# IXarea/LittleGAN

Measured on AMD Instinct MI355X. Metric: 128x128 CelebA-shaped images/sec (G+D+Adj step), higher is better.
Workload: dtype bf16; 1 GPU; C3: 128x128x3 synthetic CelebA, batch 256/GPU, bf16 MFMA conv/transposed-conv + Adjuster branch; global_batch=256, per_gpu_batch=256, image=128, cond_dim=40, parallelism=dp1, launch=eager launches

## Files before the change

### littlegan_amd/csrc/heads.hip

```cpp
#include "lg_internal.h"

namespace {

constexpr int HC_MAX = 40;

__device__ __forceinline__ float head_w(const float* __restrict__ wpr, const float* __restrict__ wc, int k, int j, int c) {
  return j == 0 ? wpr[k] : wc[(long long)k * c + (j - 1)];
}

constexpr int FS = 16;
constexpr int FKC = 256;

__global__ __launch_bounds__(256) void heads_fwd_kernel(const float* __restrict__ x, const float* __restrict__ wpr,
                                                        const float* __restrict__ wc, float* __restrict__ part, int B,
                                                        int K, int c) {
  __shared__ __attribute__((aligned(16))) float xs[FS][FKC];
  __shared__ float sred[4][FS][64];
  const int lane = threadIdx.x & 63, wid = threadIdx.x >> 6;
  const int b0 = blockIdx.y * FS, k0 = blockIdx.x * FKC;
  const bool act = lane <= c;
#pragma unroll
  for (int i = 0; i < FS * FKC / 4 / 256; ++i) {
    const int q = threadIdx.x + 256 * i, b = q / (FKC / 4), k4 = (q % (FKC / 4)) * 4;
    f32x4 v = {0.f, 0.f, 0.f, 0.f};
    if (b0 + b < B && k0 + k4 < K) v = *reinterpret_cast<const f32x4*>(x + (long long)(b0 + b) * K + k0 + k4);
    *reinterpret_cast<f32x4*>(&xs[b][k4]) = v;
  }
  __syncthreads();
  float acc[FS];
#pragma unroll
  for (int s = 0; s < FS; ++s) acc[s] = 0.f;
  const int kw = wid * 64;
#pragma unroll 2
  for (int kk = 0; kk < 64; kk += 4) {
    float w[4];
#pragma unroll
    for (int e = 0; e < 4; ++e) {
      const int k = k0 + kw + kk + e;
      w[e] = (act && k < K) ? head_w(wpr, wc, k, lane, c) : 0.f;
    }
#pragma unroll
    for (int s = 0; s < FS; ++s) {
      const f32x4 xv = *reinterpret_cast<const f32x4*>(&xs[s][kw + kk]);
      acc[s] += (xv[0] * w[0] + xv[1] * w[1]) + (xv[2] * w[2] + xv[3] * w[3]);
    }
  }
#pragma unroll
  for (int s = 0; s < FS; ++s) sred[wid][s][lane] = acc[s];
  __syncthreads();
  for (int i = threadIdx.x; i < FS * 64; i += 256) {
    const int s = i >> 6, j = i & 63;
    if (j <= c && b0 + s < B)
      part[((long long)blockIdx.x * B + b0 + s) * (c + 1) + j] = (sred[0][s][j] + sred[1][s][j]) + (sred[2][s][j] + sred[3][s][j]);
  }
}

__global__ __launch_bounds__(256) void heads_final_kernel(const float* __restrict__ part, const float* __restrict__ bpr,
                                                          const float* __restrict__ bc, float* __restrict__ p, int B,
                                                          int c, int nkc) {
  const int i = blockIdx.x * 256 + threadIdx.x;
  const int n = B * (c + 1);
  if (i >= n) return;
  const int j = i % (c + 1);
  float z = 0.f;
  for (int q = 0; q < nkc; ++q) z += part[(long long)q * n + i];
  z += j == 0 ? bpr[0] : bc[j - 1];
  p[i] = 1.f / (1.f + expf(-z));
}

constexpr int DB = 16;
__global__ __launch_bounds__(256) void heads_dgrad_kernel(const float* __restrict__ dz, const float* __restrict__ wpr,
                                                          const float* __restrict__ wc, float* __restrict__ dx, int B,
                                                          int K, int c) {
  extern __shared__ __attribute__((aligned(16))) float dsm[];
  const int cp = c | 1;
  float* sw = dsm;
  float* sdz = dsm + ((256 * cp + 3) / 4) * 4;
  const int b0 = blockIdx.y * DB, k0 = blockIdx.x * 256;
  const int kn = min(256, K - k0);
  {
    const int dq = 256 / c, dr = 256 - dq * c;
    int row = threadIdx.x / c, col = threadIdx.x - row * c;
    for (int i = threadIdx.x; i < kn * c; i += 256) {
      sw[row * cp + col] = wc[(long long)k0 * c + i];
      row += dq; col += dr;
      if (col >= c) { col -= c; ++row; }
    }
  }
  for (int i = threadIdx.x; i < DB * (c + 1); i += 256) {
    const int b = i / (c + 1), j = i - b * (c + 1);
    sdz[j * DB + b] = (b0 + b < B) ? dz[(long long)(b0 + b) * (c + 1) + j] : 0.f;
  }
  __syncthreads();
  const int k = k0 + threadIdx.x;
  if (k >= K) return;
  float acc[DB];
  const float wp = wpr[k];
#pragma unroll
  for (int q = 0; q < DB / 4; ++q) {
    const f32x4 d = *reinterpret_cast<const f32x4*>(sdz + q * 4);
#pragma unroll
    for (int e = 0; e < 4; ++e) acc[q * 4 + e] = d[e] * wp;
  }
  const float* wr = sw + threadIdx.x * cp;
  for (int j = 0; j < c; ++j) {
    const float wv = wr[j];
#pragma unroll
    for (int q = 0; q < DB / 4; ++q) {
      const f32x4 d = *reinterpret_cast<const f32x4*>(sdz + (1 + j) * DB + q * 4);
#pragma unroll
      for (int e = 0; e < 4; ++e) acc[q * 4 + e] += d[e] * wv;
    }
  }
#pragma unroll
  for (int b = 0; b < DB; ++b)
    if (b0 + b < B) dx[(long long)(b0 + b) * K + k] = acc[b];
}

constexpr int WK = 64;

__global__ __launch_bounds__(256) void heads_wgrad_kernel(const float* __restrict__ x, const float* __restrict__ dz,
                                                          float* __restrict__ dwpr, float* __restrict__ dbpr,
                                                          float* __restrict__ dwc, float* __restrict__ dbc, int B, int K,
                                                          int c, int accumulate) {
  constexpr int J = HC_MAX + 1;
  __shared__ float red[J + 1][WK + 1];
  const int lane = threadIdx.x & 63;
  const int wid = __builtin_amdgcn_readfirstlane(threadIdx.x >> 6);
  const int k0 = blockIdx.x * WK, k = k0 + lane;
  const bool kok = k < K;
  const int bq = (B + 3) / 4, bs = wid * bq, be = min(B, bs + bq);
  const bool do_bias = blockIdx.x == 0;
  float acc[J];
#pragma unroll
  for (int j = 0; j < J; ++j) acc[j] = 0.f;
  float bsum = 0.f;
  constexpr int U = 8;
  for (int b = bs; b < be; b += U) {
    float xv[U], dv[U];
#pragma unroll
    for (int u = 0; u < U; ++u) {
      const bool ok = b + u < be;
      xv[u] = (ok && kok) ? x[(long long)(b + u) * K + k] : 0.f;
      dv[u] = (ok && lane <= c) ? dz[(long long)(b + u) * (c + 1) + lane] : 0.f;
    }
#pragma unroll
    for (int u = 0; u < U; ++u) {
      bsum += dv[u];
#pragma unroll
      for (int j = 0; j < J; ++j)
        acc[j] += xv[u] * __builtin_bit_cast(float, __builtin_amdgcn_readlane(__builtin_bit_cast(int, dv[u]), j));
    }
  }
  for (int w = 0; w < 4; ++w) {
    if (wid == w) {
#pragma unroll
      for (int j = 0; j < J; ++j) red[j][lane] = (w == 0 ? 0.f : red[j][lane]) + acc[j];
      red[J][lane] = (w == 0 ? 0.f : red[J][lane]) + bsum;
    }
    __syncthreads();
  }
  if (do_bias && threadIdx.x <= c) {
    float* o = threadIdx.x == 0 ? dbpr : dbc + (threadIdx.x - 1);
    *o = (accumulate ? *o : 0.f) + red[J][threadIdx.x];
  }
  for (int i = threadIdx.x; i < WK * (c + 1); i += 256) {
    const int kk = i / (c + 1), j = i - kk * (c + 1);
    if (k0 + kk < K) {
      float* o = j == 0 ? dwpr + (k0 + kk) : dwc + (long long)(k0 + kk) * c + (j - 1);
      *o = (accumulate ? *o : 0.f) + red[j][kk];
    }
  }
}

}

extern "C" size_t lg_heads_fwd_workspace_bytes(int B, int K, int c) {
  return (size_t)lg_cdiv(K, FKC) * (size_t)B * (size_t)(c + 1) * sizeof(float);
}

extern "C" int lg_heads_fwd_partials(const float* x, const float* wpr, const float* wc, float* part, int B, int K, int c, int* nkc_out,
                                     void* stream) {
  int nkc = lg_cdiv(K, FKC);
  const int rc = lg_heads_fwd_mfma_try(x, wpr, wc, part, B, K, c, &nkc, stream);
  if (rc != LG_OK && rc != LG_ERR_UNSUPPORTED) return rc;
  if (rc == LG_ERR_UNSUPPORTED) {
    hipLaunchKernelGGL(heads_fwd_kernel, dim3(nkc, lg_cdiv(B, FS)), dim3(256), 0, (hipStream_t)stream, x, wpr, wc, part,
                       B, K, c);
    LG_CHECK_LAUNCH("lg_heads_fwd");
    lg_note_kernel("heads_fwd_kernel");
  }
  *nkc_out = nkc;
  return LG_OK;
}

extern "C" int lg_heads_fwd(const float* x, const float* wpr, const float* bpr, const float* wc, const float* bc,
                            float* p, void* workspace, size_t ws_bytes, int B, int K, int c, void* stream) {
  LG_CHECK_ARG(x && wpr && bpr && wc && bc && p && workspace, "lg_heads_fwd: null pointer");
  LG_CHECK_ARG(B > 0 && K > 0 && K % 4 == 0 && c >= 1 && c <= HC_MAX, "lg_heads_fwd: bad shape B=%d K=%d c=%d", B, K, c);
  LG_CHECK_ARG(ws_bytes >= lg_heads_fwd_workspace_bytes(B, K, c), "lg_heads_fwd: workspace too small (%zu bytes)", ws_bytes);
  int nkc = 0;
  float* part = (float*)workspace;
  const int rc = lg_heads_fwd_partials(x, wpr, wc, part, B, K, c, &nkc, stream);
  if (rc != LG_OK) return rc;
  hipLaunchKernelGGL(heads_final_kernel, dim3(lg_cdiv(B * (c + 1), 256)), dim3(256), 0, (hipStream_t)stream, part, bpr,
                     bc, p, B, c, nkc);
  LG_CHECK_LAUNCH("lg_heads_fwd(final)");
  return LG_OK;
}

extern "C" int lg_heads_dgrad(const float* dz, const float* wpr, const float* wc, float* dx, int B, int K, int c,
                              void* stream) {
  LG_CHECK_ARG(dz && wpr && wc && dx, "lg_heads_dgrad: null pointer");
  LG_CHECK_ARG(B > 0 && K > 0 && c >= 1 && c <= HC_MAX, "lg_heads_dgrad: bad shape B=%d K=%d c=%d", B, K, c);
  {
    const int rc = lg_heads_dgrad_mfma_try(dz, wpr, wc, dx, B, K, c, stream);
    if (rc != LG_ERR_UNSUPPORTED) return rc;
  }
  dim3 grid(lg_cdiv(K, 256), lg_cdiv(B, DB));
  const size_t lds = (size_t)((256 * (c | 1) + 3) / 4 * 4 + DB * (c + 1)) * sizeof(float);
  hipLaunchKernelGGL(heads_dgrad_kernel, grid, dim3(256), lds, (hipStream_t)stream, dz, wpr, wc, dx, B, K, c);
  LG_CHECK_LAUNCH("lg_heads_dgrad");
  lg_note_kernel("heads_dgrad_kernel");
  return LG_OK;
}

extern "C" int lg_heads_wgrad(const float* x, const float* dz, float* dwpr, float* dbpr, float* dwc, float* dbc, int B,
                              int K, int c, int accumulate, void* stream) {
  LG_CHECK_ARG(x && dz && dwpr && dbpr && dwc && dbc, "lg_heads_wgrad: null pointer");
  LG_CHECK_ARG(B > 0 && K > 0 && K % 4 == 0 && c >= 1 && c <= HC_MAX, "lg_heads_wgrad: bad shape B=%d K=%d c=%d", B, K, c);
  {
    const int rc = lg_heads_wgrad_mfma_try(x, dz, dwpr, dbpr, dwc, dbc, B, K, c, accumulate, stream);
    if (rc != LG_ERR_UNSUPPORTED) return rc;
  }
  hipLaunchKernelGGL(heads_wgrad_kernel, dim3(lg_cdiv(K, WK)), dim3(256), 0, (hipStream_t)stream, x, dz, dwpr, dbpr,
                     dwc, dbc, B, K, c, accumulate);
  LG_CHECK_LAUNCH("lg_heads_wgrad");
  lg_note_kernel("heads_wgrad_kernel");
  return LG_OK;
}
```

### littlegan_amd/csrc/skinny_mfma.hip

```cpp
#include <stdlib.h>
#include "lg_internal.h"

namespace {

__device__ __forceinline__ f32x16 mfma2(float a, float b, f32x16 c) { return __builtin_amdgcn_mfma_f32_32x32x2f32(a, b, c, 0, 0, 0); }
__device__ __forceinline__ f32x16 zero16() {
  f32x16 z;
#pragma unroll
  for (int e = 0; e < 16; ++e) z[e] = 0.f;
  return z;
}
struct HeadCol { const float* ptr; int stride; bool ok; };
__device__ __forceinline__ HeadCol head_col(const float* wpr, const float* wc, int j, int c) {
  HeadCol h;
  h.ok = j <= c;
  h.ptr = j == 0 ? wpr : wc + (h.ok ? j - 1 : 0);
  h.stride = j == 0 ? 1 : c;
  return h;
}

__global__ __launch_bounds__(256) void heads_fwd_mfma_kernel(const float* __restrict__ x, const float* __restrict__ wpr,
                                                             const float* __restrict__ wc, float* __restrict__ part, int B,
                                                             int K, int c) {
  __shared__ float sred[4][2][16][64];
  const int lane = threadIdx.x & 63, wid = threadIdx.x >> 6, r = lane & 31, h = lane >> 5;
  const int b0 = blockIdx.y * 32, kw = blockIdx.x * 512 + wid * 128 + 8 * h;
  const float* xr = x + (long long)(b0 + r) * K + kw;
  const HeadCol c0 = head_col(wpr, wc, r, c), c1 = head_col(wpr, wc, 32 + r, c);
  const bool two = c >= 32;
  f32x16 acc0 = zero16(), acc1 = zero16();
  constexpr int GU = 2;
  for (int g2 = 0; g2 < 8; g2 += GU) {
    f32x4 alo[GU], ahi[GU];
    float w0[GU][8], w1[GU][8];
#pragma unroll
    for (int u = 0; u < GU; ++u) {
      const int g = g2 + u;
      alo[u] = *reinterpret_cast<const f32x4*>(xr + 16 * g); ahi[u] = *reinterpret_cast<const f32x4*>(xr + 16 * g + 4);
#pragma unroll
      for (int e = 0; e < 8; ++e) {
        const long long k = kw + 16 * g + e;
        w0[u][e] = c0.ok ? c0.ptr[k * c0.stride] : 0.f;
        w1[u][e] = (two && c1.ok) ? c1.ptr[k * c1.stride] : 0.f;
      }
    }
#pragma unroll
    for (int u = 0; u < GU; ++u)
#pragma unroll
      for (int e = 0; e < 8; ++e) {
        const float a = e < 4 ? alo[u][e & 3] : ahi[u][e & 3];
        acc0 = mfma2(a, w0[u][e], acc0);
        if (two) acc1 = mfma2(a, w1[u][e], acc1);
      }
  }
#pragma unroll
  for (int e = 0; e < 16; ++e) { sred[wid][0][e][lane] = acc0[e]; sred[wid][1][e][lane] = acc1[e]; }
  __syncthreads();
  for (int i = threadIdx.x; i < 32 * 64; i += 256) {
    const int row = i >> 6, j = i & 63;
    if (j <= c) {
      const int nt = j >> 5, rr = j & 31, hh = (row >> 2) & 1, e = (row & 3) + 4 * (row >> 3), l = hh * 32 + rr;
      part[((long long)blockIdx.x * B + b0 + row) * (c + 1) + j] =
          (sred[0][nt][e][l] + sred[1][nt][e][l]) + (sred[2][nt][e][l] + sred[3][nt][e][l]);
    }
  }
}

__global__ __launch_bounds__(256) void heads_wgrad_mfma_kernel(const float* __restrict__ x, const float* __restrict__ dz,
                                                              float* __restrict__ dwpr, float* __restrict__ dbpr,
                                                              float* __restrict__ dwc, float* __restrict__ dbc, int B, int K,
                                                              int c, int accumulate) {
  __shared__ float red[2][16][64];
  __shared__ float rbias[2][64];
  const int lane = threadIdx.x & 63, wid = threadIdx.x >> 6, r = lane & 31, h = lane >> 5;
  const int k0 = blockIdx.x * 32;
  const bool ok0 = r <= c, ok1 = 32 + r <= c, two = c >= 32;
  float bs0 = 0.f, bs1 = 0.f;
  const int bq = B / 4, bs = wid * bq;
  const float* xp = x + (long long)(bs + h) * K + k0 + r;
  const float* d0 = dz + (long long)(bs + h) * (c + 1) + r;
  const float* d1 = d0 + 32;
  f32x16 acc0 = zero16(), acc1 = zero16();
  constexpr int SU = 16;
  for (int b = 0; b < bq; b += 2 * SU) {
    float a[SU], v0[SU], v1[SU];
#pragma unroll
    for (int s = 0; s < SU; ++s) {
      const bool ok = b + 2 * s < bq;
      a[s] = ok ? xp[(long long)(b + 2 * s) * K] : 0.f;
      v0[s] = (ok && ok0) ? d0[(long long)(b + 2 * s) * (c + 1)] : 0.f;
      v1[s] = (ok && two && ok1) ? d1[(long long)(b + 2 * s) * (c + 1)] : 0.f;
    }
#pragma unroll
    for (int s = 0; s < SU; ++s) {
      acc0 = mfma2(a[s], v0[s], acc0);
      if (two) acc1 = mfma2(a[s], v1[s], acc1);
      bs0 += v0[s]; bs1 += v1[s];
    }
  }
  for (int w = 0; w < 4; ++w) {
    if (wid == w) {
#pragma unroll
      for (int e = 0; e < 16; ++e) {
        red[0][e][lane] = (w == 0 ? 0.f : red[0][e][lane]) + acc0[e];
        red[1][e][lane] = (w == 0 ? 0.f : red[1][e][lane]) + acc1[e];
      }
      rbias[0][lane] = (w == 0 ? 0.f : rbias[0][lane]) + bs0;
      rbias[1][lane] = (w == 0 ? 0.f : rbias[1][lane]) + bs1;
    }
    __syncthreads();
  }
  for (int i = threadIdx.x; i < 32 * 64; i += 256) {
    const int row = i >> 6, j = i & 63;
    if (j <= c) {
      const int nt = j >> 5, rr = j & 31, hh = (row >> 2) & 1, e = (row & 3) + 4 * (row >> 3);
      const int k = k0 + row;
      float* o = j == 0 ? dwpr + k : dwc + (long long)k * c + (j - 1);
      *o = (accumulate ? *o : 0.f) + red[nt][e][hh * 32 + rr];
    }
  }
  if (blockIdx.x == 0 && threadIdx.x <= c) {
    const int j = threadIdx.x, nt = j >> 5, rr = j & 31;
    float* o = j == 0 ? dbpr : dbc + (j - 1);
    *o = (accumulate ? *o : 0.f) + (rbias[nt][rr] + rbias[nt][32 + rr]);
  }
}

__global__ __launch_bounds__(256) void heads_dgrad_mfma_kernel(const float* __restrict__ dz, const float* __restrict__ wpr,
                                                               const float* __restrict__ wc, float* __restrict__ dx, int B,
                                                               int K, int c) {
  constexpr int SMAX = 21;
  extern __shared__ float sdz[];
  const int lane = threadIdx.x & 63, wid = threadIdx.x >> 6, r = lane & 31, h = lane >> 5;
  const int kt = blockIdx.x * 128 + wid * 32;
  const int cp = (c + 1) | 1, nmt = (B / 32 - blockIdx.y + gridDim.y - 1) / gridDim.y;
  for (int t = 0; t < nmt; ++t) {
    const float* src = dz + (long long)(blockIdx.y + t * gridDim.y) * 32 * (c + 1);
    for (int i = threadIdx.x; i < 32 * (c + 1); i += 256) {
      const int row = i / (c + 1), j = i - row * (c + 1);
      sdz[(t * 32 + row) * cp + j] = src[i];
    }
  }
  float bw[SMAX];
#pragma unroll
  for (int s = 0; s < SMAX; ++s) {
    const int j = 2 * s + h;
    bw[s] = j <= c ? (j == 0 ? wpr[kt + r] : wc[(long long)(kt + r) * c + j - 1]) : 0.f;
  }
  __syncthreads();
  for (int t = 0; t < nmt; ++t) {
    const int mt = blockIdx.y + t * gridDim.y;
    const float* zr = sdz + (t * 32 + r) * cp + h;
    f32x16 acc = zero16();
#pragma unroll
    for (int s = 0; s < SMAX; ++s) acc = mfma2(2 * s + h <= c ? zr[2 * s] : 0.f, bw[s], acc);
    float* o = dx + (long long)(mt * 32 + 4 * h) * K + kt + r;
#pragma unroll
    for (int e = 0; e < 16; ++e) o[(long long)((e & 3) + 8 * (e >> 2)) * K] = acc[e];
  }
}

constexpr int SD = 72;
__global__ __launch_bounds__(256) void dense_fwd_mfma_kernel(const float* __restrict__ x, const float* __restrict__ w,
                                                             const float* __restrict__ bias, float* __restrict__ y, int B,
                                                             int K, int N) {
  extern __shared__ float sx[];
  const int lane = threadIdx.x & 63, wid = threadIdx.x >> 6, r = lane & 31, h = lane >> 5;
  const int n = blockIdx.x * 128 + wid * 32 + r, b0 = blockIdx.y * 32;
  const int nsteps = (K + 1) / 2, kp = K | 1;
  {
    const float* src = x + (long long)b0 * K;
    int row = threadIdx.x / K, col = threadIdx.x - row * K;
    const int dq = 256 / K, dr = 256 - dq * K;
    for (int i = threadIdx.x; i < 32 * K; i += 256) {
      sx[row * kp + col] = src[i];
      row += dq; col += dr;
      if (col >= K) { col -= K; ++row; }
    }
  }
  __syncthreads();
  const float* xr = sx + r * kp + h;
  const float* wp = w + (long long)h * N + n;
  const float bv = bias ? bias[n] : 0.f;
  f32x16 acc, acc2 = zero16();
#pragma unroll
  for (int e = 0; e < 16; ++e) acc[e] = bv;
#pragma unroll 4
  for (int s = 0; s < nsteps; s += 2) {
    const bool ok = 2 * s + h < K, ok2 = 2 * s + 2 + h < K;
    const float a = ok ? xr[2 * s] : 0.f, a2 = ok2 ? xr[2 * s + 2] : 0.f;
    const float b = ok ? wp[(long long)(2 * s) * N] : 0.f, b2 = ok2 ? wp[(long long)(2 * s + 2) * N] : 0.f;
    acc = mfma2(a, b, acc);
    acc2 = mfma2(a2, b2, acc2);
  }
#pragma unroll
  for (int e = 0; e < 16; ++e) acc[e] += acc2[e];
  float* o = y + (long long)(b0 + 4 * h) * N + n;
#pragma unroll
  for (int e = 0; e < 16; ++e) o[(long long)((e & 3) + 8 * (e >> 2)) * N] = acc[e];
}

template <int MT>
__global__ __launch_bounds__(256) void dense_wgrad_mfma_kernel(const float* __restrict__ x, const float* __restrict__ dy,
                                                               float* __restrict__ dw, float* __restrict__ db, int B, int K,
                                                               int N, int accumulate) {
  __shared__ float red[MT][16][64];
  __shared__ float rb[64];
  const int lane = threadIdx.x & 63, wid = threadIdx.x >> 6, r = lane & 31, h = lane >> 5;
  const int n = blockIdx.x * 32 + r;
  const int bq = B / 4, bs = wid * bq;
  f32x16 acc[MT];
#pragma unroll
  for (int m = 0; m < MT; ++m) acc[m] = zero16();
  float bsum = 0.f;
  const float* dp = dy + (long long)(bs + h) * N + n;
  const float* xp = x + (long long)(bs + h) * K + r;
  constexpr int SU = 8;
  for (int b = 0; b < bq; b += 2 * SU) {
    float d[SU], a[SU][MT];
#pragma unroll
    for (int s = 0; s < SU; ++s) {
      const bool ok = b + 2 * s < bq;
      d[s] = ok ? dp[(long long)(b + 2 * s) * N] : 0.f;
#pragma unroll
      for (int m = 0; m < MT; ++m) a[s][m] = (ok && 32 * m + r < K) ? xp[(long long)(b + 2 * s) * K + 32 * m] : 0.f;
    }
#pragma unroll
    for (int s = 0; s < SU; ++s) {
      bsum += d[s];
#pragma unroll
      for (int m = 0; m < MT; ++m) acc[m] = mfma2(a[s][m], d[s], acc[m]);
    }
  }
  for (int w = 0; w < 4; ++w) {
    if (wid == w) {
#pragma unroll
      for (int m = 0; m < MT; ++m)
#pragma unroll
        for (int e = 0; e < 16; ++e) red[m][e][lane] = (w == 0 ? 0.f : red[m][e][lane]) + acc[m][e];
      rb[lane] = (w == 0 ? 0.f : rb[lane]) + bsum;
    }
    __syncthreads();
  }
  for (int i = threadIdx.x; i < MT * 32 * 32; i += 256) {
    const int k = i >> 5, rr = i & 31;
    if (k < K) {
      const int m = k >> 5, row = k & 31, hh = (row >> 2) & 1, e = (row & 3) + 4 * (row >> 3);
      float* o = dw + (long long)k * N + blockIdx.x * 32 + rr;
      *o = (accumulate ? *o : 0.f) + red[m][e][hh * 32 + rr];
    }
  }
  if (db && threadIdx.x < 32) {
    float* o = db + blockIdx.x * 32 + threadIdx.x;
    *o = (accumulate ? *o : 0.f) + (rb[threadIdx.x] + rb[32 + threadIdx.x]);
  }
}

bool skinny_on() {
  static int on = -1;
  if (on < 0) on = lg_env_flag("LG_NO_SKINNY_MFMA") ? 0 : 1;
  return on == 1;
}

}

extern "C" int lg_heads_fwd_mfma_try(const float* x, const float* wpr, const float* wc, float* part, int B, int K, int c,
                                     int* nkc_out, void* stream) {
  if (!skinny_on() || B % 32 || K % 512 || c < 1 || c > 40) return LG_ERR_UNSUPPORTED;
  hipLaunchKernelGGL(heads_fwd_mfma_kernel, dim3(K / 512, B / 32), dim3(256), 0, (hipStream_t)stream, x, wpr, wc, part, B, K, c);
  LG_CHECK_LAUNCH("lg_heads_fwd(mfma)");
  lg_note_kernel("heads_fwd_mfma_kernel");
  *nkc_out = K / 512;
  return LG_OK;
}

extern "C" int lg_heads_wgrad_mfma_try(const float* x, const float* dz, float* dwpr, float* dbpr, float* dwc, float* dbc, int B,
                                       int K, int c, int accumulate, void* stream) {
  if (!skinny_on() || B % 64 || K % 32 || c < 1 || c > 40) return LG_ERR_UNSUPPORTED;
  hipLaunchKernelGGL(heads_wgrad_mfma_kernel, dim3(K / 32), dim3(256), 0, (hipStream_t)stream, x, dz, dwpr, dbpr, dwc, dbc, B, K, c,
                     accumulate);
  LG_CHECK_LAUNCH("lg_heads_wgrad(mfma)");
  lg_note_kernel("heads_wgrad_mfma_kernel");
  return LG_OK;
}

extern "C" int lg_heads_dgrad_mfma_try(const float* dz, const float* wpr, const float* wc, float* dx, int B, int K, int c,
                                       void* stream) {
  if (!skinny_on() || B % 32 || K % 128 || c < 1 || c > 40) return LG_ERR_UNSUPPORTED;
  const int mt = B / 32, gy = mt >= 8 ? 4 : (mt >= 2 ? 2 : 1);
  const size_t lds = (size_t)((mt + gy - 1) / gy) * 32 * ((c + 1) | 1) * sizeof(float);
  if (lds > 48 * 1024) return LG_ERR_UNSUPPORTED;
  hipLaunchKernelGGL(heads_dgrad_mfma_kernel, dim3(K / 128, gy), dim3(256), lds, (hipStream_t)stream, dz, wpr, wc, dx, B, K, c);
  LG_CHECK_LAUNCH("lg_heads_dgrad(mfma)");
  lg_note_kernel("heads_dgrad_mfma_kernel");
  return LG_OK;
}

extern "C" int lg_dense_fwd_mfma_try(const float* x, const float* w, const float* bias, float* y, int B, int K, int N,
                                     void* stream) {
  if (!skinny_on() || B % 32 || N % 128 || K < 1 || K > 2 * SD) return LG_ERR_UNSUPPORTED;
  hipLaunchKernelGGL(dense_fwd_mfma_kernel, dim3(N / 128, B / 32), dim3(256), (size_t)32 * (K | 1) * sizeof(float),
                     (hipStream_t)stream, x, w, bias, y, B, K, N);
  LG_CHECK_LAUNCH("lg_dense_fwd(mfma)");
  lg_note_kernel("dense_fwd_mfma_kernel");
  return LG_OK;
}

extern "C" int lg_dense_wgrad_mfma_try(const float* x, const float* dy, float* dw, float* db, int B, int K, int N, int accumulate,
                                       void* stream) {
  if (!skinny_on() || B % 32 || N % 32 || K < 1 || K > 160) return LG_ERR_UNSUPPORTED;
  const int mt = (K + 31) / 32;
  hipStream_t st = (hipStream_t)stream;
  const dim3 grid(N / 32);
#define LG_DW(M) hipLaunchKernelGGL(dense_wgrad_mfma_kernel<M>, grid, dim3(256), 0, st, x, dy, dw, db, B, K, N, accumulate)
  if (mt == 1) LG_DW(1); else if (mt == 2) LG_DW(2); else if (mt == 3) LG_DW(3); else if (mt == 4) LG_DW(4); else LG_DW(5);
#undef LG_DW
  LG_CHECK_LAUNCH("lg_dense_wgrad(mfma)");
  lg_note_kernel(mt == 1 ? "dense_wgrad_mfma_kernel<1>" : mt == 2 ? "dense_wgrad_mfma_kernel<2>" : mt == 3 ? "dense_wgrad_mfma_kernel<3>"
                 : mt == 4 ? "dense_wgrad_mfma_kernel<4>" : "dense_wgrad_mfma_kernel<5>");
  return LG_OK;
}
```

Measured before the change: 24760 images/sec.

## Persist dense_fwd MFMA weights in registers and pipeline batch tiles via LDS

The dense forward MFMA kernel is templated on K padding and now loads each block's weight column slice into registers once. It then loops over several 32-row batch tiles using double-buffered LDS, prefetching the next x tile into registers while the current tile is computed. The grid is capped at about 768 blocks and an occupancy hint is added. Separately, the heads final reduction over K-chunks is unrolled by 16 so more independent loads are in flight. The cost is more register pressure, and the vectorized f32x4 x loads assume 16-byte alignment and K*8 row layout.

```diff
diff --git a/littlegan_amd/csrc/heads.hip b/littlegan_amd/csrc/heads.hip
--- a/littlegan_amd/csrc/heads.hip
+++ b/littlegan_amd/csrc/heads.hip
@@ -63,7 +63,17 @@
   if (i >= n) return;
   const int j = i % (c + 1);
   float z = 0.f;
-  for (int q = 0; q < nkc; ++q) z += part[(long long)q * n + i];
+  const float* pp = part + i;
+  int q = 0;
+  constexpr int U = 16;
+  for (; q + U <= nkc; q += U) {
+    float v[U];
+#pragma unroll
+    for (int u = 0; u < U; ++u) v[u] = pp[(long long)(q + u) * n];
+#pragma unroll
+    for (int u = 0; u < U; ++u) z += v[u];
+  }
+  for (; q < nkc; ++q) z += pp[(long long)q * n];
   z += j == 0 ? bpr[0] : bc[j - 1];
   p[i] = 1.f / (1.f + expf(-z));
 }
diff --git a/littlegan_amd/csrc/skinny_mfma.hip b/littlegan_amd/csrc/skinny_mfma.hip
--- a/littlegan_amd/csrc/skinny_mfma.hip
+++ b/littlegan_amd/csrc/skinny_mfma.hip
@@ -161,43 +161,71 @@
 }
 
 constexpr int SD = 72;
-__global__ __launch_bounds__(256) void dense_fwd_mfma_kernel(const float* __restrict__ x, const float* __restrict__ w,
+constexpr int XQ = 5;
+template <int NP>
+__global__ __launch_bounds__(256) __attribute__((amdgpu_waves_per_eu(3))) void dense_fwd_mfma_kernel(const float* __restrict__ x, const float* __restrict__ w,
                                                              const float* __restrict__ bias, float* __restrict__ y, int B,
                                                              int K, int N) {
+  static_assert(2 * NP <= SD, "K <= 144");
   extern __shared__ float sx[];
-  const int lane = threadIdx.x & 63, wid = threadIdx.x >> 6, r = lane & 31, h = lane >> 5;
-  const int n = blockIdx.x * 128 + wid * 32 + r, b0 = blockIdx.y * 32;
-  const int nsteps = (K + 1) / 2, kp = K | 1;
-  {
-    const float* src = x + (long long)b0 * K;
-    int row = threadIdx.x / K, col = threadIdx.x - row * K;
-    const int dq = 256 / K, dr = 256 - dq * K;
-    for (int i = threadIdx.x; i < 32 * K; i += 256) {
-      sx[row * kp + col] = src[i];
-      row += dq; col += dr;
-      if (col >= K) { col -= K; ++row; }
-    }
-  }
-  __syncthreads();
-  const float* xr = sx + r * kp + h;
-  const float* wp = w + (long long)h * N + n;
+  constexpr int kp = 4 * NP + 3;
+  const int lane = threadIdx.x & 63, wid = threadIdx.x >> 6, r = lane & 31, h = lane >> 5;
+  const int n = blockIdx.x * 128 + wid * 32 + r;
+  const int nq = 8 * K;
+  const int nmt = (B / 32 - blockIdx.y + gridDim.y - 1) / gridDim.y;
+  f32x4 xq[XQ];
+  auto fetch = [&](int mt) {
+    const f32x4* src = reinterpret_cast<const f32x4*>(x + (long long)mt * 32 * K);
+#pragma unroll
+    for (int q = 0; q < XQ; ++q) {
+      const int i = threadIdx.x + 256 * q;
+      if (i < nq) xq[q] = src[i];
+    }
+  };
+  fetch(blockIdx.y);
+  float bw[2 * NP];
+#pragma unroll
+  for (int s = 0; s < 2 * NP; ++s) {
+    const int ks = 2 * s < K ? 2 * s : K - 1;
+    const bool ok = 2 * s + h < K;
+    const float v = (w + (long long)ks * N)[(ks + h < K ? (unsigned)(h * N) : 0u) + (unsigned)n];
+    bw[s] = ok ? v : 0.f;
+  }
+  for (int i = threadIdx.x; i < 64 * (kp - K); i += 256) sx[i / (kp - K) * kp + K + i % (kp - K)] = 0.f;
   const float bv = bias ? bias[n] : 0.f;
-  f32x16 acc, acc2 = zero16();
-#pragma unroll
-  for (int e = 0; e < 16; ++e) acc[e] = bv;
-#pragma unroll 4
-  for (int s = 0; s < nsteps; s += 2) {
-    const bool ok = 2 * s + h < K, ok2 = 2 * s + 2 + h < K;
-    const float a = ok ? xr[2 * s] : 0.f, a2 = ok2 ? xr[2 * s + 2] : 0.f;
-    const float b = ok ? wp[(long long)(2 * s) * N] : 0.f, b2 = ok2 ? wp[(long long)(2 * s + 2) * N] : 0.f;
-    acc = mfma2(a, b, acc);
-    acc2 = mfma2(a2, b2, acc2);
-  }
-#pragma unroll
-  for (int e = 0; e < 16; ++e) acc[e] += acc2[e];
-  float* o = y + (long long)(b0 + 4 * h) * N + n;
-#pragma unroll
-  for (int e = 0; e < 16; ++e) o[(long long)((e & 3) + 8 * (e >> 2)) * N] = acc[e];
+  for (int t = 0; t < nmt; ++t) {
+    const int mt = blockIdx.y + t * gridDim.y;
+    float* buf = sx + (t & 1) * 32 * kp;
+#pragma unroll
+    for (int q = 0; q < XQ; ++q) {
+      const int i = threadIdx.x + 256 * q;
+      if (i < nq) {
+        int row = 4 * i / K, col = 4 * i - row * K;
+#pragma unroll
+        for (int e = 0; e < 4; ++e) {
+          while (col >= K) { col -= K; ++row; }
+          buf[row * kp + col] = xq[q][e];
+          ++col;
+        }
+      }
+    }
+    __syncthreads();
+    if (t + 1 < nmt) fetch(mt + gridDim.y);
+    const float* xr = buf + r * kp + h;
+    f32x16 acc, acc2 = zero16();
+#pragma unroll
+    for (int e = 0; e < 16; ++e) acc[e] = bv;
+#pragma unroll
+    for (int s = 0; s < 2 * NP; s += 2) {
+      acc = mfma2(xr[2 * s], bw[s], acc);
+      acc2 = mfma2(xr[2 * s + 2], bw[s + 1], acc2);
+    }
+#pragma unroll
+    for (int e = 0; e < 16; ++e) acc[e] += acc2[e];
+    float* o = y + (long long)(mt * 32 + 4 * h) * N + n;
+#pragma unroll
+    for (int e = 0; e < 16; ++e) o[(long long)((e & 3) + 8 * (e >> 2)) * N] = acc[e];
+  }
 }
 
 template <int MT>
@@ -299,8 +327,11 @@
 extern "C" int lg_dense_fwd_mfma_try(const float* x, const float* w, const float* bias, float* y, int B, int K, int N,
                                      void* stream) {
   if (!skinny_on() || B % 32 || N % 128 || K < 1 || K > 2 * SD) return LG_ERR_UNSUPPORTED;
-  hipLaunchKernelGGL(dense_fwd_mfma_kernel, dim3(N / 128, B / 32), dim3(256), (size_t)32 * (K | 1) * sizeof(float),
-                     (hipStream_t)stream, x, w, bias, y, B, K, N);
+  const int mt = B / 32, nb = N / 128, gy = mt < (768 + nb - 1) / nb ? mt : (768 + nb - 1) / nb;
+  hipStream_t st = (hipStream_t)stream;
+#define LG_DF(P) hipLaunchKernelGGL(dense_fwd_mfma_kernel<P>, dim3(nb, gy), dim3(256), (size_t)2 * 32 * (4 * P + 3) * sizeof(float), st, x, w, bias, y, B, K, N)
+  if (K <= 40) LG_DF(10); else if (K <= 80) LG_DF(20); else if (K <= 136) LG_DF(34); else LG_DF(36);
+#undef LG_DF
   LG_CHECK_LAUNCH("lg_dense_fwd(mfma)");
   lg_note_kernel("dense_fwd_mfma_kernel");
   return LG_OK;
```

New measurement: 24830 images/sec, median of 6. No clear change (+0.3%).
